# axiom-crypto/halo2-lib

Hardware: AMD Instinct MI355X
Metric: create_proof constraints/sec (k=19 ECDSA configuration, halo2-ecc/configs/secp256k1/bench_ecdsa.config:1); MSM G1-adds/sec in `msm_2_20` (higher is better)
Workload: dtype u32 (254-bit Montgomery integers as 8x32 / 9x29-bit limbs); 1 GPU; BASELINE configs[3]: h2hip_plonk_create_proof, k=19 secp256k1-ECDSA shape (bench_ecdsa.config:1: 1 advice + 1 lookup + 1 constants column, lookup_bits 18), synthetic circuit-like witness resident in HBM; 1 step = 1 proof, bytes back on the host; constraints_per_proof=524280, msm_count=12, msm_size=524288, extended_k=21, degree=5, proof_bytes=960

## Files before the change

### halo2-lib_amd/csrc/capi.hip

```cpp
#include <stdarg.h>

#include <algorithm>

#include "internal.h"
#include <sched.h>

namespace h2 {

static thread_local char g_err[512] = "";

void set_error(const char *fmt, ...) {
    va_list ap;
    va_start(ap, fmt);
    vsnprintf(g_err, sizeof(g_err), fmt, ap);
    va_end(ap);
}

int ws_reserve(h2hip_ctx *ctx, int slot, size_t bytes, void **out) {
    DevBuf &b = ctx->ws[slot];
    if (bytes == 0) bytes = 256;
    if (b.cap < bytes) {
        if (b.p) {
            H2_HIPCHK(hipStreamSynchronize(ctx->stream));
            if (ctx->clean_stream) H2_HIPCHK(hipStreamSynchronize(ctx->clean_stream));
// ... 135 lines not shown
    ctx->pending.clear();
}

static void prof_collect_all(h2hip_ctx *ctx);
void prof_fold_child(h2hip_ctx *parent, h2hip_ctx *child) {
    prof_collect(child);
    for (auto &kv : child->stats) {
        parent->stats[kv.first].total_ms += kv.second.total_ms;
        parent->stats[kv.first].launches += kv.second.launches;
        parent->stats[kv.first].spans.insert(parent->stats[kv.first].spans.end(), kv.second.spans.begin(), kv.second.spans.end());
    }
    child->stats.clear();
}
static void prof_collect_all(h2hip_ctx *ctx) {
    prof_collect(ctx);
    for (h2hip_ctx *l : ctx->lane)
        if (l) prof_fold_child(ctx, l);
}

}

using namespace h2;

extern "C" {

const char *h2hip_last_error(void) { return g_err; }
int h2hip_version(void) { return 100; }

int h2hip_device_count(int *count) {
    H2_REQUIRE(count, "count is NULL");
    int n = 0;
    hipError_t e = hipGetDeviceCount(&n);
    if (e != hipSuccess) {
        *count = 0;
        set_error("hipGetDeviceCount failed: %s", hipGetErrorString(e));
        return H2HIP_ERR_NO_DEVICE;
    }
    *count = n;
    return H2HIP_OK;
}

int h2hip_init(int device, void *hip_stream, h2hip_ctx **out) {
    H2_REQUIRE(out, "out is NULL");
    *out = nullptr;
    int n = 0;
    if (hipGetDeviceCount(&n) != hipSuccess || n <= 0) {
        set_error("no HIP device available (libh2hip has no CPU fallback)");
        return H2HIP_ERR_NO_DEVICE;
    }
    H2_REQUIRE(device >= 0 && device < n, "device index out of range");
    H2_HIPCHK(hipSetDevice(device));
    h2hip_ctx *ctx = new h2hip_ctx();
    ctx->device = device;
    hipDeviceProp_t prop;
    if (hipGetDeviceProperties(&prop, device) == hipSuccess) ctx->num_cus = prop.multiProcessorCount;
    if (hip_stream) {
        ctx->stream = (hipStream_t)hip_stream;
        ctx->own_stream = false;
    } else {
        hipError_t e = hipStreamCreateWithFlags(&ctx->stream, hipStreamNonBlocking);
        if (e != hipSuccess) {
            set_error("hipStreamCreate failed: %s", hipGetErrorString(e));
            delete ctx;
            return H2HIP_ERR_HIP;
        }
        ctx->own_stream = true;
    }
    *out = ctx;
    return H2HIP_OK;
}

}
namespace h2 {
constexpr size_t JOB_RING_BYTES = (size_t)1 << 20;
int upload_jobs(h2hip_ctx *ctx, void *dst_dev, const void *src_host, size_t bytes) {
    if (!bytes) return H2HIP_OK;
    if (bytes > JOB_RING_BYTES / 4) {
        H2_HIPCHK(hipMemcpyAsync(dst_dev, src_host, bytes, hipMemcpyHostToDevice, ctx->stream));
        H2_HIPCHK(hipStreamSynchronize(ctx->stream));
        return H2HIP_OK;
    }
    if (!ctx->job_ring) H2_HIPCHK(hipHostMalloc((void **)&ctx->job_ring, JOB_RING_BYTES, 0));
    const size_t need = (bytes + 255) / 256 * 256;
    if (ctx->job_ring_off + need > JOB_RING_BYTES) {
        H2_HIPCHK(hipStreamSynchronize(ctx->stream));
        ctx->job_ring_off = 0;
    }
    char *slot = ctx->job_ring + ctx->job_ring_off;
    memcpy(slot, src_host, bytes);
    ctx->job_ring_off += need;
    H2_HIPCHK(hipMemcpyAsync(dst_dev, slot, bytes, hipMemcpyHostToDevice, ctx->stream));
    return H2HIP_OK;
}
}
extern "C" {

void h2hip_destroy(h2hip_ctx *ctx) {
    if (!ctx) return;
    hipSetDevice(ctx->device);
    hipStreamSynchronize(ctx->stream);
    for (int l = 0; l < 4; ++l)
        if (ctx->lane[l]) hipStreamSynchronize(ctx->lane[l]->stream);
    if (ctx->clean_stream) {
        hipStreamSynchronize(ctx->clean_stream);
        hipStreamDestroy(ctx->clean_stream);
        hipEventDestroy(ctx->clean_ev);
        hipEventDestroy(ctx->clean_ev1);
        hipEventDestroy(ctx->used_ev);
    }
    if (ctx->tail_ev) hipEventDestroy(ctx->tail_ev);
    if (ctx->sorted_ev) hipEventDestroy(ctx->sorted_ev);
    if (ctx->job_ring) hipHostFree(ctx->job_ring);
    if (ctx->poll_host) hipHostFree(ctx->poll_host);
    for (auto &b : ctx->ws)
        if (b.p) hipFree(b.p);
    for (auto &t : ctx->twiddles) {
        hipFree(t.t1);
        hipFree(t.t2);
        for (int k = 0; k < 4; ++k) {
            if (t.direct[k]) hipFree(t.direct[k]);
        }
    }
    for (auto &p : ctx->pending) {
        hipEventDestroy(p.begin);
        hipEventDestroy(p.end);
    }
    for (auto e : ctx->event_pool) hipEventDestroy(e);
    if (ctx->prof_ref && ctx->own_prof_ref) hipEventDestroy(ctx->prof_ref);
    for (int l = 0; l < 4; ++l)
        if (ctx->lane[l]) {
            h2hip_destroy(ctx->lane[l]);
            hipEventDestroy(ctx->lane_ev[l]);
        }
    if (ctx->fork_ev) hipEventDestroy(ctx->fork_ev);
    if (ctx->fork_ev2) hipEventDestroy(ctx->fork_ev2);
    if (ctx->fork_ev3) hipEventDestroy(ctx->fork_ev3);
    for (auto e : ctx->timer_ev)
        if (e) hipEventDestroy(e);
    if (ctx->own_stream) hipStreamDestroy(ctx->stream);
    delete ctx;
}

int h2hip_sync(h2hip_ctx *ctx) {
    H2_DEVICE_GUARD(ctx);
    H2_REQUIRE(ctx, "ctx is NULL");
    H2_HIPCHK(hipStreamSynchronize(ctx->stream));
    return H2HIP_OK;
}

static int *param_slot(h2hip_ctx *ctx, const char *name) {
#define H2_KNOB_SLOT(knob, inherit, legal, domain) \
    if (!strcmp(name, #knob)) return &ctx->knob;
    H2_KNOB_TABLE(H2_KNOB_SLOT)
#undef H2_KNOB_SLOT
    return nullptr;
}
int h2hip_set_param(h2hip_ctx *ctx, const char *name, int value) {
    H2_DEVICE_GUARD(ctx);
    H2_REQUIRE(ctx && name, "NULL argument");
    int *p = param_slot(ctx, name);
    H2_REQUIRE(p, "unknown parameter name");
#define H2_KNOB_CHECK(knob, inherit, legal, domain)                                                     \
    if (p == &ctx->knob) {                                                                              \
        const int v = value;                                                                            \
        if (!(legal)) {                                                                                 \
            set_error("h2hip_set_param: invalid argument: " #knob " = %d: must be " domain, value);   \
            return H2HIP_ERR_INVALID;                                                                   \
        }                                                                                               \
    }
    H2_KNOB_TABLE(H2_KNOB_CHECK)
#undef H2_KNOB_CHECK
    *p = value;
    return H2HIP_OK;
}
int h2hip_get_param(h2hip_ctx *ctx, const char *name, int *value) {
    H2_DEVICE_GUARD(ctx);
    H2_REQUIRE(ctx && name && value, "NULL argument");
    int *p = param_slot(ctx, name);
    H2_REQUIRE(p, "unknown parameter name");
    *value = *p;
    return H2HIP_OK;
}

int h2hip_malloc(h2hip_ctx *ctx, size_t bytes, void **dptr) {
    H2_DEVICE_GUARD(ctx);
    H2_REQUIRE(ctx && dptr, "NULL argument");
    hipError_t e = hipMalloc(dptr, bytes ? bytes : 256);
    if (e != hipSuccess) {
        set_error("hipMalloc(%zu) failed: %s", bytes, hipGetErrorString(e));
        return H2HIP_ERR_NOMEM;
    }
    return H2HIP_OK;
}
int h2hip_free(h2hip_ctx *ctx, void *dptr) {
    H2_DEVICE_GUARD(ctx);
    H2_REQUIRE(ctx, "ctx is NULL");
    if (!dptr) return H2HIP_OK;
    H2_HIPCHK(hipStreamSynchronize(ctx->stream));
    H2_HIPCHK(hipFree(dptr));
    return H2HIP_OK;
}
int h2hip_host_register(h2hip_ctx *ctx, void *host_ptr, size_t bytes) {
    H2_DEVICE_GUARD(ctx);
    H2_REQUIRE(ctx && host_ptr && bytes, "NULL argument");
    H2_HIPCHK(hipHostRegister(host_ptr, bytes, hipHostRegisterDefault));
    return H2HIP_OK;
}
int h2hip_host_unregister(h2hip_ctx *ctx, void *host_ptr) {
    H2_DEVICE_GUARD(ctx);
    H2_REQUIRE(ctx && host_ptr, "NULL argument");
    H2_HIPCHK(hipHostUnregister(host_ptr));
    return H2HIP_OK;
}
int h2hip_upload(h2hip_ctx *ctx, void *dst_dev, const void *src_host, size_t bytes) {
    H2_DEVICE_GUARD(ctx);
    H2_REQUIRE(ctx && (bytes == 0 || (dst_dev && src_host)), "NULL argument");
    if (!bytes) return H2HIP_OK;
    H2_HIPCHK(hipMemcpyAsync(dst_dev, src_host, bytes, hipMemcpyHostToDevice, ctx->stream));
    H2_HIPCHK(hipStreamSynchronize(ctx->stream));
    return H2HIP_OK;
}
int h2hip_download(h2hip_ctx *ctx, void *dst_host, const void *src_dev, size_t bytes) {
    H2_DEVICE_GUARD(ctx);
    H2_REQUIRE(ctx && (bytes == 0 || (dst_host && src_dev)), "NULL argument");
    if (!bytes) return H2HIP_OK;
    H2_HIPCHK(hipMemcpyAsync(dst_host, src_dev, bytes, hipMemcpyDeviceToHost, ctx->stream));
    H2_HIPCHK(hipStreamSynchronize(ctx->stream));
    return H2HIP_OK;
}

int h2hip_profile_enable(h2hip_ctx *ctx, int on) {
    H2_DEVICE_GUARD(ctx);
    H2_REQUIRE(ctx, "ctx is NULL");
    prof_collect_all(ctx);
    ctx->profiling = on != 0;
    return H2HIP_OK;
}
int h2hip_profile_filter(h2hip_ctx *ctx, const char *prefix) {
    H2_DEVICE_GUARD(ctx);
    H2_REQUIRE(ctx, "ctx is NULL");
    prof_collect_all(ctx);
    ctx->prof_filter = prefix ? prefix : "";
    return H2HIP_OK;
}
int h2hip_profile_reset(h2hip_ctx *ctx) {
    H2_DEVICE_GUARD(ctx);
    H2_REQUIRE(ctx, "ctx is NULL");
    prof_collect_all(ctx);
    ctx->stats.clear();
    if (!ctx->prof_ref) {
        H2_HIPCHK(hipEventCreate(&ctx->prof_ref));
        ctx->own_prof_ref = true;
    }
    if (ctx->own_prof_ref) {
        H2_HIPCHK(hipEventRecord(ctx->prof_ref, ctx->stream));
        H2_HIPCHK(hipEventSynchronize(ctx->prof_ref));
    }
    return H2HIP_OK;
}
int h2hip_profile_get_busy(h2hip_ctx *ctx, const char *prefix, double *busy_ms) {
    H2_DEVICE_GUARD(ctx);
    H2_REQUIRE(ctx && prefix && busy_ms, "NULL argument");
    prof_collect_all(ctx);
    std::vector<std::pair<float, float>> all;
    size_t len = strlen(prefix);
    for (auto &kv : ctx->stats)
        if (kv.first.compare(0, len, prefix) == 0) all.insert(all.end(), kv.second.spans.begin(), kv.second.spans.end());
    std::sort(all.begin(), all.end());
    double busy = 0;
    float cur0 = 0, cur1 = -1;
    for (auto &sp : all) {
        if (cur1 < cur0 || sp.first > cur1) {
            if (cur1 >= cur0) busy += cur1 - cur0;
            cur0 = sp.first;
            cur1 = sp.second;
        } else if (sp.second > cur1) {
            cur1 = sp.second;
        }
    }
    if (cur1 >= cur0) busy += cur1 - cur0;
    *busy_ms = busy;
    return H2HIP_OK;
}
int h2hip_profile_get(h2hip_ctx *ctx, const char *prefix, double *total_ms, uint64_t *launches) {
    H2_DEVICE_GUARD(ctx);
    H2_REQUIRE(ctx && prefix, "NULL argument");
    prof_collect_all(ctx);
    double ms = 0;
    uint64_t cnt = 0;
    size_t len = strlen(prefix);
    for (auto &kv : ctx->stats)
        if (kv.first.compare(0, len, prefix) == 0) {
            ms += kv.second.total_ms;
            cnt += kv.second.launches;
        }
    if (total_ms) *total_ms = ms;
    if (launches) *launches = cnt;
    return H2HIP_OK;
}
int h2hip_profile_dump(h2hip_ctx *ctx, char *out, size_t cap, size_t *needed) {
    H2_DEVICE_GUARD(ctx);
    H2_REQUIRE(ctx && (out || cap == 0), "NULL argument");
    prof_collect_all(ctx);
    std::string text;
    for (auto &kv : ctx->stats) {
        std::vector<std::pair<float, float>> all(kv.second.spans.begin(), kv.second.spans.end());
        std::sort(all.begin(), all.end());
        double busy = 0;
        float cur0 = 0, cur1 = -1;
        for (auto &sp : all) {
            if (cur1 < cur0 || sp.first > cur1) {
                if (cur1 >= cur0) busy += cur1 - cur0;
                cur0 = sp.first;
                cur1 = sp.second;
            } else if (sp.second > cur1) {
                cur1 = sp.second;
            }
        }
        if (cur1 >= cur0) busy += cur1 - cur0;
        char line[256];
        snprintf(line, sizeof(line), "%s %.6f %llu %.6f\n", kv.first.c_str(), kv.second.total_ms, (unsigned long long)kv.second.launches, busy);
        text += line;
    }
// ... 31 lines not shown
```

### halo2-lib_amd/csrc/fr_ops.hip

```cpp
#include "internal.h"
#include "fr29.cuh"
#include "fq29.cuh"

namespace h2 {


enum { OP_ADD = 0, OP_SUB = 1, OP_MUL = 2 };

template <int OP>
__global__ __launch_bounds__(256) void fr_binop_kernel(Fr *__restrict__ out, const Fr *__restrict__ a, const Fr *__restrict__ b, size_t n) {
    size_t stride = (size_t)gridDim.x * blockDim.x;
    for (size_t i = (size_t)blockIdx.x * blockDim.x + threadIdx.x; i < n; i += stride) {
        Fr x = a[i], y = b[i];
        out[i] = OP == OP_ADD ? fe_add(x, y) : OP == OP_SUB ? fe_sub(x, y) : fe_mul(x, y);
    }
}

__global__ __launch_bounds__(256) void fr_mul_add_kernel(Fr *__restrict__ out, const Fr *__restrict__ a, const Fr *__restrict__ b,
                                                         const Fr *__restrict__ c, size_t n) {
    size_t stride = (size_t)gridDim.x * blockDim.x;
    for (size_t i = (size_t)blockIdx.x * blockDim.x + threadIdx.x; i < n; i += stride) out[i] = fe_add(fe_mul(a[i], b[i]), c[i]);
}

__global__ __launch_bounds__(256) void fr_axpby_kernel(Fr *__restrict__ y, Fr s, bool scale_y, const Fr *__restrict__ x, Fr a, size_t n) {
    size_t stride = (size_t)gridDim.x * blockDim.x;
    for (size_t i = (size_t)blockIdx.x * blockDim.x + threadIdx.x; i < n; i += stride) {
        Fr v = y[i];
        if (scale_y) v = fe_mul(v, s);
        if (x) v = fe_add(v, fe_mul(a, x[i]));
        y[i] = v;
    }
}

constexpr uint32_t LINCOMB_MAX = 15;
struct LinCombArgs {
    const Fr *p[LINCOMB_MAX];
    Fr29 c[LINCOMB_MAX];
    uint32_t count, accumulate;
};
__global__ __launch_bounds__(256) void fr_lincomb_kernel(Fr *out, LinCombArgs a, size_t n) {
    const size_t stride = (size_t)gridDim.x * blockDim.x;
    for (size_t i = (size_t)blockIdx.x * blockDim.x + threadIdx.x; i < n; i += stride) {
        Fr29 tot = a.accumulate ? f29_split<R29P>(out[i]) : Fr29::zero();
        for (uint32_t j0 = 0; j0 < a.count; j0 += 5) {
            Fr29 x[5], c[5];
#pragma unroll
            for (uint32_t t = 0; t < 5; ++t) {
                const bool live = j0 + t < a.count;
                x[t] = live ? f29_split<R29P>(a.p[j0 + t][i]) : Fr29::zero();
                c[t] = live ? a.c[j0 + t] : Fr29::zero();
            }
            tot = f29_add(tot, f29_dot<5>(x, c));
        }
        out[i] = f29_pack_canonical<FrP>(f29_weak_reduce(f29_norm(tot)));
    }
}

__global__ __launch_bounds__(256) void fr_batch_invert_kernel(const Fr *src, Fr *dst, Fr *__restrict__ scratch, size_t n) {
    const size_t T = (size_t)gridDim.x * blockDim.x, t = (size_t)blockIdx.x * blockDim.x + threadIdx.x;
    if (t >= n) return;
    Fr acc = Fr::one();
    size_t last = t;
    for (size_t i = t; i < n; i += T) {
        Fr v = src[i];
        scratch[i] = acc;
        if (!v.is_zero()) acc = fe_mul(acc, v);
        last = i;
    }
    Fr inv = fe_inv(acc);
    for (size_t i = last;; i -= T) {
        Fr v = src[i];
        if (!v.is_zero()) {
            dst[i] = fe_mul(inv, scratch[i]);
            inv = fe_mul(inv, v);
        } else if (dst != src) {
            dst[i] = v;
        }
        if (i < T) break;
    }
}


constexpr uint32_t SCAN_J = 8;
__global__ __launch_bounds__(256) void fr_prefix_prod_tile_kernel(const Fr *__restrict__ in, Fr *__restrict__ out, Fr *__restrict__ tile_prod,
                                                                  size_t n, size_t seg_stride) {
    __shared__ Fr sh[256];
    in += (size_t)blockIdx.y * seg_stride;
    out += (size_t)blockIdx.y * seg_stride;
    tile_prod += (size_t)blockIdx.y * gridDim.x;
    const uint32_t tid = threadIdx.x;
    const size_t base = ((size_t)blockIdx.x * 256 + tid) * SCAN_J;
    Fr acc = Fr::one();
    for (uint32_t k = 0; k < SCAN_J; ++k)
        if (base + k < n) acc = fe_mul(acc, in[base + k]);
    sh[tid] = acc;
    __syncthreads();
    for (uint32_t d = 1; d < 256; d <<= 1) {
        Fr o = Fr::one();
        if (tid >= d) o = sh[tid - d];
        __syncthreads();
        if (tid >= d) sh[tid] = fe_mul(sh[tid], o);
        __syncthreads();
    }
    Fr run = tid ? sh[tid - 1] : Fr::one();
    for (uint32_t k = 0; k < SCAN_J; ++k)
        if (base + k < n) {
            run = fe_mul(run, in[base + k]);
            out[base + k] = run;
        }
    if (tid == 255) tile_prod[blockIdx.x] = sh[255];
}
__global__ __launch_bounds__(1024) void fr_prefix_prod_sums_kernel(Fr *__restrict__ tile_prod, uint32_t ntiles) {
    __shared__ Fr sh[1024];
    tile_prod += (size_t)blockIdx.x * ntiles;
    const uint32_t tid = threadIdx.x;
    const uint32_t per = (ntiles + 1023) / 1024, lo = tid * per, hi = lo + per < ntiles ? lo + per : ntiles;
    Fr acc = Fr::one();
    for (uint32_t k = lo; k < hi; ++k) acc = fe_mul(acc, tile_prod[k]);
    sh[tid] = acc;
    __syncthreads();
    for (uint32_t d = 1; d < 1024; d <<= 1) {
        Fr o = Fr::one();
        if (tid >= d) o = sh[tid - d];
        __syncthreads();
        if (tid >= d) sh[tid] = fe_mul(sh[tid], o);
        __syncthreads();
    }
    Fr run = tid ? sh[tid - 1] : Fr::one();
    for (uint32_t k = lo; k < hi; ++k) {
        Fr t = tile_prod[k];
        tile_prod[k] = run;
        run = fe_mul(run, t);
    }
}
__global__ __launch_bounds__(256) void fr_prefix_prod_apply_kernel(Fr *__restrict__ out, const Fr *__restrict__ tile_excl, size_t n, size_t seg_stride) {
    const size_t base = ((size_t)blockIdx.x * 256 + threadIdx.x) * SCAN_J;
    if (blockIdx.x == 0) return;
    out += (size_t)blockIdx.y * seg_stride;
    Fr m = tile_excl[(size_t)blockIdx.y * gridDim.x + blockIdx.x];
    for (uint32_t k = 0; k < SCAN_J; ++k)
        if (base + k < n) out[base + k] = fe_mul(out[base + k], m);
}
__global__ __launch_bounds__(256) void fr_set_one_kernel(Fr *__restrict__ z) {
    if (threadIdx.x == 0 && blockIdx.x == 0) z[0] = Fr::one();
}
__global__ __launch_bounds__(256) void fr_ratio_rows_kernel(Fr *__restrict__ r, const Fr *__restrict__ num, const Fr *__restrict__ den_inv, size_t total,
                                                            size_t seg_len, int chained) {
    const size_t stride = (size_t)gridDim.x * blockDim.x;
    for (size_t g = (size_t)blockIdx.x * blockDim.x + threadIdx.x; g < total; g += stride) {
        const size_t seg = g / seg_len, i = g - seg * seg_len;
        const size_t dst = chained ? g + 1 : seg * (seg_len + 1) + i + 1;
        r[dst] = fe_mul(num[g], den_inv[g]);
        if (i == 0 && (!chained || seg == 0)) r[dst - 1] = Fr::one();
    }
}
struct RowPtrs {
    Fr *p[32];
};
__global__ __launch_bounds__(256) void fr_scatter_rows_kernel(RowPtrs dst, const Fr *__restrict__ src, size_t src_stride, size_t len) {
    Fr *__restrict__ d = dst.p[blockIdx.y];
    const Fr *__restrict__ sp = src + (size_t)blockIdx.y * src_stride;
    const size_t stride = (size_t)gridDim.x * blockDim.x;
    for (size_t i = (size_t)blockIdx.x * blockDim.x + threadIdx.x; i < len; i += stride) d[i] = sp[i];
}

}

using namespace h2;

extern "C" {

static int binop(h2hip_ctx *ctx, int op, void *out, const void *a, const void *b, size_t n) {
    H2_REQUIRE(ctx && (n == 0 || (out && a && b)), "NULL argument");
    if (!n) return H2HIP_OK;
    dim3 g(grid_for(ctx, n)), blk(256);
    prof_begin(ctx, "fr_binop_kernel");
    if (op == OP_ADD) hipLaunchKernelGGL(fr_binop_kernel<OP_ADD>, g, blk, 0, ctx->stream, (Fr *)out, (const Fr *)a, (const Fr *)b, n);
    if (op == OP_SUB) hipLaunchKernelGGL(fr_binop_kernel<OP_SUB>, g, blk, 0, ctx->stream, (Fr *)out, (const Fr *)a, (const Fr *)b, n);
    if (op == OP_MUL) hipLaunchKernelGGL(fr_binop_kernel<OP_MUL>, g, blk, 0, ctx->stream, (Fr *)out, (const Fr *)a, (const Fr *)b, n);
    prof_end(ctx);
    H2_HIPCHK(hipGetLastError());
    return H2HIP_OK;
}
int h2hip_fr_add_batch_dev(h2hip_ctx *ctx, void *out, const void *a, const void *b, size_t n) {
    H2_DEVICE_GUARD(ctx); return binop(ctx, OP_ADD, out, a, b, n); }
int h2hip_fr_sub_batch_dev(h2hip_ctx *ctx, void *out, const void *a, const void *b, size_t n) {
    H2_DEVICE_GUARD(ctx); return binop(ctx, OP_SUB, out, a, b, n); }
int h2hip_fr_mul_batch_dev(h2hip_ctx *ctx, void *out, const void *a, const void *b, size_t n) {
    H2_DEVICE_GUARD(ctx); return binop(ctx, OP_MUL, out, a, b, n); }
int h2hip_fr_mul_add_batch_dev(h2hip_ctx *ctx, void *out, const void *a, const void *b, const void *c, size_t n) {
    H2_DEVICE_GUARD(ctx);
    H2_REQUIRE(ctx && (n == 0 || (out && a && b && c)), "NULL argument");
    if (!n) return H2HIP_OK;
    prof_begin(ctx, "fr_mul_add_kernel");
    hipLaunchKernelGGL(fr_mul_add_kernel, dim3(grid_for(ctx, n)), dim3(256), 0, ctx->stream, (Fr *)out, (const Fr *)a, (const Fr *)b,
                       (const Fr *)c, n);
    prof_end(ctx);
    H2_HIPCHK(hipGetLastError());
    return H2HIP_OK;
}
int h2hip_fr_axpy_dev(h2hip_ctx *ctx, void *y, const void *a, const void *x, size_t n) {
    H2_DEVICE_GUARD(ctx);
    H2_REQUIRE(ctx && a && (n == 0 || (y && x)), "NULL argument");
    if (!n) return H2HIP_OK;
    Fr av;
    memcpy(&av, a, sizeof(Fr));
    prof_begin(ctx, "fr_axpby_kernel");
    hipLaunchKernelGGL(fr_axpby_kernel, dim3(grid_for(ctx, n)), dim3(256), 0, ctx->stream, (Fr *)y, Fr::one(), false, (const Fr *)x, av, n);
    prof_end(ctx);
    H2_HIPCHK(hipGetLastError());
    return H2HIP_OK;
}
int h2hip_fr_axpby_dev(h2hip_ctx *ctx, void *y, const void *s, const void *a, const void *x, size_t n) {
    H2_DEVICE_GUARD(ctx);
    H2_REQUIRE(ctx && a && s && (n == 0 || (y && x)), "NULL argument");
    if (!n) return H2HIP_OK;
    Fr av, sv;
    memcpy(&av, a, sizeof(Fr));
    memcpy(&sv, s, sizeof(Fr));
    prof_begin(ctx, "fr_axpby_kernel");
    hipLaunchKernelGGL(fr_axpby_kernel, dim3(grid_for(ctx, n)), dim3(256), 0, ctx->stream, (Fr *)y, sv, true, (const Fr *)x, av, n);
    prof_end(ctx);
    H2_HIPCHK(hipGetLastError());
    return H2HIP_OK;
}
int h2hip_fr_scale_dev(h2hip_ctx *ctx, void *y, const void *s, size_t n) {
    H2_DEVICE_GUARD(ctx);
    H2_REQUIRE(ctx && s && (n == 0 || y), "NULL argument");
    if (!n) return H2HIP_OK;
    Fr sv;
    memcpy(&sv, s, sizeof(Fr));
    prof_begin(ctx, "fr_axpby_kernel");
    hipLaunchKernelGGL(fr_axpby_kernel, dim3(grid_for(ctx, n)), dim3(256), 0, ctx->stream, (Fr *)y, sv, true, (const Fr *)nullptr, Fr::one(), n);
    prof_end(ctx);
    H2_HIPCHK(hipGetLastError());
    return H2HIP_OK;
}

int h2hip_fr_linear_combination_dev(h2hip_ctx *ctx, void *out, const void *const *polys, const void *coeffs, size_t count, size_t n) {
    H2_DEVICE_GUARD(ctx);
    H2_REQUIRE(ctx && (n == 0 || out) && (count == 0 || (polys && coeffs)), "NULL argument");
    if (!n) return H2HIP_OK;
    for (size_t j = 0; j < count; ++j) H2_REQUIRE(polys[j], "NULL polynomial");
    if (!count) {
        H2_HIPCHK(hipMemsetAsync(out, 0, sizeof(Fr) * n, ctx->stream));
        return H2HIP_OK;
    }
    const Fr *cs = (const Fr *)coeffs;
    for (size_t j0 = 0; j0 < count; j0 += LINCOMB_MAX) {
        LinCombArgs a;
        a.count = (uint32_t)(count - j0 < LINCOMB_MAX ? count - j0 : LINCOMB_MAX);
        a.accumulate = j0 ? 1u : 0u;
        for (uint32_t t = 0; t < LINCOMB_MAX; ++t) {
            const bool live = t < a.count;
            Fr c;
            if (live) memcpy(&c, cs + j0 + t, sizeof(Fr));
            a.p[t] = live ? (const Fr *)polys[j0 + t] : nullptr;
            a.c[t] = live ? fr29_from_sat(c) : Fr29::zero();
        }
        prof_begin(ctx, "fr_lincomb_kernel");
        hipLaunchKernelGGL(fr_lincomb_kernel, dim3(grid_for(ctx, n)), dim3(256), 0, ctx->stream, (Fr *)out, a, n);
        prof_end(ctx);
    }
    H2_HIPCHK(hipGetLastError());
    return H2HIP_OK;
}

}
namespace h2 {
int fr_batch_invert_to(h2hip_ctx *ctx, const Fr *src, Fr *dst, size_t n) {
    if (!n) return H2HIP_OK;
    Fr *scratch = nullptr;
    H2_CHK(ws_reserve(ctx, h2hip_ctx::WS_TMP1, sizeof(Fr) * n, (void **)&scratch));
    size_t per_lane = (size_t)ctx->fr_invert_run;
    if (per_lane < 1) {
        per_lane = n >> 16;
        per_lane = per_lane < 4 ? 4 : per_lane > 32 ? 32 : per_lane;
    }
    size_t lanes = (n + per_lane - 1) / per_lane;
    uint32_t blocks = (uint32_t)((lanes + 255) / 256);
    prof_begin(ctx, "fr_batch_invert_kernel");
    hipLaunchKernelGGL(fr_batch_invert_kernel, dim3(blocks), dim3(256), 0, ctx->stream, src, dst, scratch, n);
    prof_end(ctx);
    H2_HIPCHK(hipGetLastError());
    return H2HIP_OK;
}
}
extern "C" {
int h2hip_fr_batch_invert_dev(h2hip_ctx *ctx, void *a, size_t n) {
    H2_DEVICE_GUARD(ctx);
    H2_REQUIRE(ctx && (n == 0 || a), "NULL argument");
    return fr_batch_invert_to(ctx, (const Fr *)a, (Fr *)a, n);
}

static int prefix_product_segments(h2hip_ctx *ctx, const Fr *in, Fr *out, size_t n, size_t segments, size_t seg_stride) {
    const uint32_t tile = 256 * SCAN_J;
    uint32_t ntiles = (uint32_t)((n + tile - 1) / tile);
    H2_REQUIRE(segments >= 1 && segments <= 65535, "1..65535 segments");
    Fr *tp = nullptr;
    H2_CHK(ws_reserve(ctx, h2hip_ctx::WS_TMP2, sizeof(Fr) * ((size_t)ntiles * segments + 1), (void **)&tp));
    prof_begin(ctx, "fr_prefix_prod_kernels");
    hipLaunchKernelGGL(fr_prefix_prod_tile_kernel, dim3(ntiles, (uint32_t)segments), dim3(256), 0, ctx->stream, in, out, tp, n, seg_stride);
    hipLaunchKernelGGL(fr_prefix_prod_sums_kernel, dim3((uint32_t)segments), dim3(1024), 0, ctx->stream, tp, ntiles);
    hipLaunchKernelGGL(fr_prefix_prod_apply_kernel, dim3(ntiles, (uint32_t)segments), dim3(256), 0, ctx->stream, out, (const Fr *)tp, n, seg_stride);
    prof_end(ctx);
    H2_HIPCHK(hipGetLastError());
    return H2HIP_OK;
}
static int prefix_product_inplace(h2hip_ctx *ctx, const Fr *in, Fr *out, size_t n) { return prefix_product_segments(ctx, in, out, n, 1, 0); }
}
namespace h2 {
int fr_scatter_rows(h2hip_ctx *ctx, Fr *const *dst, size_t count, const Fr *src, size_t src_stride, size_t len) {
    if (!count || !len) return H2HIP_OK;
    prof_begin(ctx, "fr_scatter_rows_kernel");
    for (size_t s0 = 0; s0 < count; s0 += 32) {
        const uint32_t g = (uint32_t)(count - s0 < 32 ? count - s0 : 32);
        RowPtrs rows;
        for (uint32_t j = 0; j < 32; ++j) rows.p[j] = dst[s0 + (j < g ? j : 0)];
        hipLaunchKernelGGL(fr_scatter_rows_kernel, dim3(grid_for(ctx, len), g), dim3(256), 0, ctx->stream, rows, src + s0 * src_stride, src_stride, len);
    }
    prof_end(ctx);
    H2_HIPCHK(hipGetLastError());
    return H2HIP_OK;
}
}
extern "C" {
int h2hip_fr_prefix_product_dev(h2hip_ctx *ctx, void *out, const void *in, size_t n) {
    H2_DEVICE_GUARD(ctx);
    H2_REQUIRE(ctx && (n == 0 || (out && in)), "NULL argument");
    if (!n) return H2HIP_OK;
    return prefix_product_inplace(ctx, (const Fr *)in, (Fr *)out, n);
}
int h2hip_fr_grand_product_dev(h2hip_ctx *ctx, void *z, const void *num, const void *den, size_t n) {
    H2_DEVICE_GUARD(ctx);
    H2_REQUIRE(ctx && z && (n == 0 || (num && den)), "NULL argument");
    Fr *zz = (Fr *)z;
    hipLaunchKernelGGL(fr_set_one_kernel, dim3(1), dim3(64), 0, ctx->stream, zz);
    if (!n) return H2HIP_OK;
    Fr *t = nullptr;
    H2_CHK(ws_reserve(ctx, h2hip_ctx::WS_TMP0, sizeof(Fr) * n, (void **)&t));
    H2_CHK(fr_batch_invert_to(ctx, (const Fr *)den, t, n));
    H2_CHK(binop(ctx, OP_MUL, t, t, num, n));
    return prefix_product_inplace(ctx, t, zz + 1, n);
}

int h2hip_fr_grand_products_dev(h2hip_ctx *ctx, void *const *z, const void *num, const void *den, size_t segments, size_t seg_len, int chained) {
    H2_DEVICE_GUARD(ctx);
    H2_REQUIRE(ctx && (segments == 0 || z) && (segments == 0 || seg_len == 0 || (num && den)), "NULL argument");
    if (!segments) return H2HIP_OK;
    for (size_t s2 = 0; s2 < segments; ++s2) H2_REQUIRE(z[s2], "NULL product column");
    H2_REQUIRE(segments <= 65535 && seg_len < ((size_t)1 << 40), "too many segments");
    const size_t total = segments * seg_len;
    const size_t rlen = chained ? total + 1 : segments * (seg_len + 1);
    Fr *t = nullptr, *r = nullptr;
    H2_CHK(ws_reserve(ctx, h2hip_ctx::WS_TMP0, sizeof(Fr) * (total + 2 * rlen), (void **)&t));
    r = t + total;
    Fr *e = r + rlen;
    if (!total) {
        for (size_t s2 = 0; s2 < segments; ++s2) hipLaunchKernelGGL(fr_set_one_kernel, dim3(1), dim3(64), 0, ctx->stream, (Fr *)z[s2]);
        H2_HIPCHK(hipGetLastError());
        return H2HIP_OK;
    }
    H2_CHK(fr_batch_invert_to(ctx, (const Fr *)den, t, total));
    prof_begin(ctx, "fr_ratio_rows_kernel");
    hipLaunchKernelGGL(fr_ratio_rows_kernel, dim3(grid_for(ctx, total)), dim3(256), 0, ctx->stream, r, (const Fr *)num, (const Fr *)t, total, seg_len,
                       chained ? 1 : 0);
    prof_end(ctx);
    if (segments == 1) return prefix_product_segments(ctx, r, (Fr *)z[0], rlen, 1, 0);
    if (chained) H2_CHK(prefix_product_segments(ctx, r, e, rlen, 1, 0));
    else H2_CHK(prefix_product_segments(ctx, r, e, seg_len + 1, segments, seg_len + 1));
    return fr_scatter_rows(ctx, (Fr *const *)z, segments, e, chained ? seg_len : seg_len + 1, seg_len + 1);
}

}
```

### halo2-lib_amd/csrc/internal.h

```cpp
#pragma once
#include <hip/hip_runtime.h>
#include <stdint.h>
#include <stdio.h>
#include <string.h>
#include <functional>
#include <map>
#include <string>
#include <vector>

#include "../../include/h2hip.h"
#include "ec.cuh"
#include "ec29.cuh"

namespace h2 {

void set_error(const char *fmt, ...);

#define H2_HIPCHK(expr)                                                                              \
    do {                                                                                             \
        hipError_t e__ = (expr);                                                                     \
        if (e__ != hipSuccess) {                                                                     \
            h2::set_error("%s:%d: %s -> %s", __FILE__, __LINE__, #expr, hipGetErrorString(e__));     \
            return H2HIP_ERR_HIP;                                                                    \
        }                                                                                            \
    } while (0)

#define H2_CHK(expr)                      \
    do {                                  \
        int r__ = (expr);                 \
        if (r__ != H2HIP_OK) return r__;  \
    } while (0)

#define H2_REQUIRE_AS(func, cond, msg)                           \
    do {                                                         \
        if (!(cond)) {                                           \
            h2::set_error("%s: invalid argument: %s", func, msg); \
            return H2HIP_ERR_INVALID;                            \
        }                                                        \
    } while (0)
#define H2_REQUIRE(cond, msg) H2_REQUIRE_AS(__func__, cond, msg)

struct DevBuf {
    void *p = nullptr;
    size_t cap = 0;
};

struct TwiddleSet {
    uint32_t log_n = 0, lo_bits = 0;
    Fr omega;
    void *t1 = nullptr;
    void *t2 = nullptr;
    void *direct[4] = {nullptr, nullptr, nullptr, nullptr};
    uint32_t direct_log_s[4] = {0, 0, 0, 0};
};

struct KernelStat {
    double total_ms = 0;
    uint64_t launches = 0;
    std::vector<std::pair<float, float>> spans;
};

}

struct h2hip_ctx {
    int device = 0;
    hipStream_t stream = nullptr;
    bool own_stream = false;
    int num_cus = 256;
    enum { WS_NTT = 0, WS_DIGITS, WS_COUNTS, WS_OFFSETS, WS_CURSOR, WS_SKEY, WS_SVAL, WS_BUCKETS, WS_PKEY0, WS_PVAL0, WS_PKEY1,
           WS_PVAL1, WS_SEG, WS_WIN, WS_OUT, WS_SCAN, WS_TMP0, WS_TMP1, WS_TMP2, WS_STAGE, WS_POSEIDON, WS_FBTABLE, WS_BATCH, WS_LK0, WS_LK1, WS_LK2, WS_LK3, WS_LK4, WS_LK5, WS_VANISH, WS_BATCH_BUCKETS, WS_COUNT };
    h2::DevBuf ws[WS_COUNT];
    std::vector<h2::TwiddleSet> twiddles;
    uint32_t pos_t = 0, pos_rf = 0, pos_rp = 0;
    bool msm_lds_attr_set = false, lookup_lds_attr_set = false, ntt_lds_attr_set = false;
    int msm_window_bits = 0;
    int msm_chunk = 0;
    int msm_chunk_lone = -1;
    int msm_seg = 4;
    int msm_quad_tails = 1;
    int msm_quad_seg_max = 32768;
    int msm_sort_threads = 1024;
    int msm_sort_groups = 0;
    int msm_hist_split = 0;
    int msm_hist_packed = 1;
    int msm_scatter_split = 0;
    int msm_scatter_full_lds = 0;
    int msm_table_split = 1;
    int msm_lanes = 0;
    int msm_stagger_sorts = -1;
    int msm_fuse_cols = 0;
    int msm_defer_reduce = 1;
    int clean_on_lane = 1;
    int ntt_tile_bits = 10;
    int ntt_min_col_bits = 2;
    int ntt_full_table = 1;
    int ntt_tile_kernel = 1;
    int ntt_debug_skip = 0;
    int quotient_29 = 1;
    int kate_29 = 1;
    int kate_coeffs_per_lane = 0;
    int fr_invert_run = 0;
    int lookup_big_tile_bits = 19;
    int host_poll = 1;
#ifdef H2_HIPEMU
    int plonk_warm_keygen = 0;
#else
    int plonk_warm_keygen = 1;
#endif
    int plonk_tail_overlap = 1;
    int plonk_side_on_lanes = 1;
    int plonk_permute_in_commit = 1;
    int plonk_merge_products = 1;
    int plonk_shard_side = 1;
    int plonk_route_rows = 1;
    int plonk_lazy_upload = 1;
    int plonk_early_intt = 1;
    int plonk_gate_before_join = 0;
    bool is_lane = false;
    h2hip_ctx *lane[4] = {nullptr, nullptr, nullptr, nullptr};
    hipEvent_t lane_ev[4] = {nullptr, nullptr, nullptr, nullptr};
    hipEvent_t sorted_ev = nullptr;
    char *job_ring = nullptr;
    size_t job_ring_off = 0;
    hipEvent_t fork_ev = nullptr, fork_ev2 = nullptr, fork_ev3 = nullptr, tail_ev = nullptr;
    hipStream_t clean_stream = nullptr;
    hipEvent_t clean_ev = nullptr, clean_ev1 = nullptr, used_ev = nullptr;
    void *clean_ptr[2] = {nullptr, nullptr};
    size_t clean_bytes[2] = {0, 0};
    hipEvent_t timer_ev[2] = {nullptr, nullptr};
    char *poll_host = nullptr;
    char *poll_dev = nullptr;
    unsigned long long poll_seq = 0;
    bool profiling = false;
    std::string prof_filter;
    std::map<std::string, h2::KernelStat> stats;
    struct PendingLaunch {
        std::string name;
        hipEvent_t begin, end;
        bool ended;
    };
    std::vector<PendingLaunch> pending;
    std::vector<hipEvent_t> event_pool;
    hipEvent_t prof_ref = nullptr;
    bool own_prof_ref = false;
};

namespace h2 {
inline bool knob_pow2(int v) { return v > 0 && (v & (v - 1)) == 0; }
}
#define H2_INHERITED true
#define H2_PARENT_ONLY(why) false
#define H2_KNOB_TABLE(K)                                                                                                                          \
    K(msm_window_bits, H2_INHERITED, v == 0 || (v >= 4 && v <= 16), "0 (auto) or 4..16")                                                         \
    K(msm_chunk, H2_INHERITED, v == 0 || (v >= 2 && v <= 4096), "0 (auto) or 2..4096")                                                          \
    K(msm_chunk_lone, H2_INHERITED, v >= -1 && v <= 4096, "-1 (auto), 0 (the batch rule) or 1..4096")                                          \
    K(msm_seg, H2_INHERITED, h2::knob_pow2(v) && v <= 1024, "a power of two <= 1024")                                                          \
    K(msm_quad_tails, H2_INHERITED, v == 0 || v == 1, "0 or 1")                                                                                 \
    K(msm_quad_seg_max, H2_INHERITED, v >= 0, ">= 0")                                                                                           \
    K(msm_sort_threads, H2_INHERITED, v == 256 || v == 512 || v == 1024, "256, 512 or 1024")                                                   \
    K(msm_sort_groups, H2_INHERITED, v >= 0 && v <= 1024, "0 (auto) or 1..1024")                                                               \
    K(msm_hist_split, H2_INHERITED, v == 0 || (h2::knob_pow2(v) && v <= 64), "0 or a power of two <= 64")                                      \
    K(msm_hist_packed, H2_INHERITED, v == 0 || v == 1, "0 or 1")                                                                                \
    K(msm_scatter_split, H2_INHERITED, v == 0 || (h2::knob_pow2(v) && v <= 64), "0 (auto) or a power of two <= 64")                            \
    K(msm_scatter_full_lds, H2_INHERITED, v == 0 || v == 1, "0 or 1")                                                                           \
    K(msm_table_split, H2_INHERITED, v == 0 || v == 1, "0 or 1")                                                                                \
    K(msm_lanes, H2_PARENT_ONLY("read only by the batch driver, on the caller's context"), v >= 0 && v <= 4, "0 (auto) or 1..4")              \
    K(msm_stagger_sorts, H2_PARENT_ONLY("read only by the batch driver, on the caller's context"), v >= -1 && v <= 1, "-1 (auto), 0 or 1")     \
    K(msm_fuse_cols, H2_PARENT_ONLY("read only by the batch driver, on the caller's context"), v >= 0 && v <= (int)h2::MSM_MAX_COLS,           \
      "0 (auto) or 1..32")                                                                                                                        \
    K(msm_defer_reduce, H2_PARENT_ONLY("read only by the batch driver, on the caller's context"), v == 0 || v == 1, "0 or 1")                  \
    K(clean_on_lane, H2_PARENT_ONLY("read only by the batch driver, on the caller's context"), v == 0 || v == 1, "0 or 1")                     \
    K(ntt_tile_bits, H2_INHERITED, v >= 4 && v <= 10, "4..10")                                                                                  \
    K(ntt_min_col_bits, H2_INHERITED, v >= 0 && v <= 5, "0..5")                                                                                 \
    K(ntt_full_table, H2_INHERITED, v == 0 || v == 1, "0 or 1")                                                                                 \
    K(ntt_tile_kernel, H2_INHERITED, v == 0 || v == 1, "0 or 1")                                                                                \
    K(ntt_debug_skip, H2_INHERITED, v >= 0 && v <= 2, "0, 1 or 2")                                                                              \
    K(quotient_29, H2_INHERITED, v == 0 || v == 1, "0 or 1")                                                                                    \
    K(kate_29, H2_INHERITED, v == 0 || v == 1, "0 or 1")                                                                                        \
    K(kate_coeffs_per_lane, H2_INHERITED, v == 0 || v == 1 || v == 2 || v == 4 || v == 8, "0 (by length), 1, 2, 4 or 8")                       \
    K(fr_invert_run, H2_INHERITED, v >= 0 && v <= 1024, "0 (auto) or 1..1024")                                                                 \
    K(lookup_big_tile_bits, H2_INHERITED, v >= 12 && v <= 28, "12..28")                                                                         \
    K(host_poll, H2_INHERITED, v == 0 || v == 1, "0 or 1")                                                                                      \
    K(plonk_warm_keygen, H2_PARENT_ONLY("read only by h2hip_plonk_keygen"), v == 0 || v == 1, "0 or 1")                                       \
    K(plonk_tail_overlap, H2_PARENT_ONLY("read only by create_proof, on the caller's context"), v == 0 || v == 1, "0 or 1")                    \
    K(plonk_side_on_lanes, H2_PARENT_ONLY("read only by create_proof, on the caller's context"), v == 0 || v == 1, "0 or 1")                   \
    K(plonk_permute_in_commit, H2_PARENT_ONLY("read only by create_proof, on the caller's context"), v == 0 || v == 1, "0 or 1")               \
    K(plonk_merge_products, H2_PARENT_ONLY("read only by create_proof, on the caller's context"), v == 0 || v == 1, "0 or 1")                  \
    K(plonk_shard_side, H2_PARENT_ONLY("read only by create_proof, on the caller's context"), v >= 0 && v <= 2, "0, 1 or 2 (forced)")          \
    K(plonk_route_rows, H2_PARENT_ONLY("read only by create_proof, on the caller's context"), v == 0 || v == 1, "0 or 1")                      \
    K(plonk_lazy_upload, H2_PARENT_ONLY("read only by create_proof, on the caller's context"), v == 0 || v == 1, "0 or 1")                     \
    K(plonk_early_intt, H2_PARENT_ONLY("read only by create_proof, on the caller's context"), v == 0 || v == 1, "0 or 1")                      \
    K(plonk_gate_before_join, H2_PARENT_ONLY("read only by create_proof, on the caller's context"), v == 0 || v == 1, "0 or 1")

namespace h2 {
inline void inherit_knobs(h2hip_ctx *c, const h2hip_ctx *p) {
#define H2_KNOB_INHERIT(name, inherit, legal, domain) \
    if (inherit) c->name = p->name;
    H2_KNOB_TABLE(H2_KNOB_INHERIT)
#undef H2_KNOB_INHERIT
    c->profiling = p->profiling;
    c->prof_filter = p->prof_filter;
    c->prof_ref = p->prof_ref;
}
struct DeviceGuard {
    int prev = -1;
    bool switched = false;
    explicit DeviceGuard(const h2hip_ctx *c) {
        if (c && hipGetDevice(&prev) == hipSuccess && prev != c->device) switched = hipSetDevice(c->device) == hipSuccess;
    }
    ~DeviceGuard() {
        if (switched) hipSetDevice(prev);
    }
    DeviceGuard(const DeviceGuard &) = delete;
    DeviceGuard &operator=(const DeviceGuard &) = delete;
};
}
#define H2_DEVICE_GUARD(ctx) h2::DeviceGuard device_guard__(ctx)

struct h2hip_bases {
    h2::G1Affine *pts = nullptr;
    h2::G1Affine *pts29 = nullptr;
    bool split = false;
    size_t n = 0;
    uint32_t window_bits = 0;
    uint32_t tables = 1;
};

namespace h2 {
struct alignas(128) TableEntry29 {
    uint32_t x[9], y[9];
    uint32_t pad[14];
};
static_assert(sizeof(TableEntry29) == 128, "one entry per 128-byte line");
int ws_reserve(h2hip_ctx *ctx, int slot, size_t bytes, void **out);
inline uint32_t grid_for(const h2hip_ctx *ctx, size_t n, size_t per_lane = 1) {
    size_t blocks = (n / per_lane + 255) / 256, cap = (size_t)ctx->num_cus * 8;
    if (blocks > cap) blocks = cap;
    return (uint32_t)(blocks ? blocks : 1);
}
inline Fr ld_fr(const void *p) {
    Fr r;
    memcpy(&r, p, sizeof(Fr));
    return r;
}
struct OmegaTable;
int ntt_pow_table(h2hip_ctx *ctx, uint32_t log_n, const Fr &omega, OmegaTable *out);

void prof_begin(h2hip_ctx *ctx, const char *name);
void prof_end(h2hip_ctx *ctx);
bool prof_launch_events(h2hip_ctx *ctx, const char *name, hipEvent_t *start, hipEvent_t *stop);

int ntt_run(h2hip_ctx *ctx, Fr *a, uint32_t log_n, const Fr &omega, const Fr *in_override, uint64_t in_len, const Fr *in_scale3,
            const Fr *out_scale3);
int ntt_run_batch(h2hip_ctx *ctx, Fr *const *a, const Fr *const *in_override, size_t ncols, uint32_t log_n, const Fr &omega, uint64_t in_len,
                  const Fr *in_scale3, const Fr *out_scale3);
constexpr uint32_t LK_COMPRESS_MAX_EXPRS = 49, LK_COMPRESS_MAX_WIDTH = 5;
int lookup_compress_batch_dev(h2hip_ctx *ctx, const Fr *const *cols, Fr *const *out, uint32_t count, uint32_t width, size_t rows, const Fr &theta);
int fr_scatter_rows(h2hip_ctx *ctx, Fr *const *dst, size_t count, const Fr *src, size_t src_stride, size_t len);
int upload_jobs(h2hip_ctx *ctx, void *dst_dev, const void *src_host, size_t bytes);
int exclusive_scan_u32_segments(h2hip_ctx *ctx, const uint32_t *in, uint32_t *out, uint32_t n, uint32_t segments, size_t in_stride,
                                size_t out_stride);
int exclusive_scan_u32(h2hip_ctx *ctx, const uint32_t *in, uint32_t *out, uint32_t n);
int batch_normalize_jac(h2hip_ctx *ctx, const G1Jac *tmp, G1Affine *out, uint32_t n);
int msm_prepare_bases(h2hip_ctx *ctx, h2hip_bases *bases, bool precompute);
int msm_run(h2hip_ctx *ctx, const h2hip_bases *bases, const Fr *scalars_dev, size_t n, XYZZ *out_dev);
constexpr uint32_t MSM_MAX_COLS = 32;
int msm_run_cols(h2hip_ctx *ctx, const h2hip_bases *bases, const Fr *const *scalars_dev, uint32_t ncols, size_t n, XYZZ *out_dev,
                 XYZZ29 *ext_buckets, bool ext_buckets_zeroed = false, hipEvent_t sorted_ev = nullptr);
struct BatchMsmHooks {
    std::function<int(size_t)> col;
    std::function<int()> mid;
    size_t mid_after = 0;
    std::function<int(hipEvent_t ev)> tail;
};
int msm_batch(h2hip_ctx *ctx, const h2hip_bases *bases, const h2hip_bases *const *bases_per_col, const void *const *scalars_in, bool scalars_on_host,
              size_t n, size_t count, int point_format, void *out_host, const BatchMsmHooks *hooks);
bool buckets_prezeroed(h2hip_ctx *ctx, int which, const void *buf, size_t bytes);
int buckets_clean_after_use(h2hip_ctx *ctx, int which, void *buf, size_t bytes, hipStream_t on = nullptr);
int sync_stream(h2hip_ctx *ctx);
int sync_results(h2hip_ctx *ctx, void *dst_host, const void *src_dev, size_t bytes);
void prof_fold_child(h2hip_ctx *parent, h2hip_ctx *child);
int rng_chacha_fill_dev(h2hip_ctx *ctx, Fr *out_dev, size_t n, const uint8_t seed[32], int rounds, uint64_t first_block, hipStream_t stream);
int comm_reserve_allgather_dev(h2hip_comm *comm, size_t bytes);
int comm_reserve_alltoall_dev(h2hip_comm *c, size_t bytes);
int plonk_phased_layout(const h2hip_phased_circuit_params &pp, h2hip_plonk_shape *shape, std::vector<std::vector<int>> *phase_cols,
                        uint32_t challenges[H2HIP_MAX_PHASE], bool *phased, h2hip_base_circuit_params *bp, const h2hip_rlc_circuit_params *rlc = nullptr);
int msm_reduce_cols(h2hip_ctx *ctx, const h2hip_bases *bases, uint32_t window_bits, const XYZZ29 *buckets, uint32_t ncols, XYZZ *out_dev);
uint32_t lookup_padded_keys(uint32_t u);
int lookup_sort_keys_dev(h2hip_ctx *ctx, void *keys, uint32_t N);
struct WitnessCheckJob {
    uint32_t u = 0;
    std::vector<const Fr *> cols;
    std::vector<uint32_t> gate_adv, gate_q;
    std::vector<uint32_t> gate_report;
    uint32_t num_rlc_gates = 0;
    Fr rlc_gamma;
    std::vector<uint32_t> lk_in, lk_q;
    const void *table_sorted = nullptr;
    uint32_t dyn_width = 0;
    std::vector<uint32_t> dyn_in, dyn_tab;
    uint32_t num_lookups = 0;
    std::vector<uint32_t> perm_col;
    const uint16_t *sigma_c = nullptr;
    const uint32_t *sigma_r = nullptr;
};
constexpr uint32_t WC_NONE = 0xFFFFFFFFu;
int witness_check_run(h2hip_ctx *ctx, const WitnessCheckJob &job, h2hip_witness_failure *failures_out, size_t max_failures, size_t *num_failures);
}
```

Before: 38.66 million constraints/s.

## Fuse grand-product computation into tiled three-pass scan with per-tile inversion

Replaces the batch-invert, ratio and prefix-product pipeline for segmented grand products with three kernels. The first computes per-tile products of numerator and denominator, the second scans the tile totals and inverts only one denominator per thread, and the third rebuilds the row products in registers and shared memory and writes them straight into the product columns. This cuts full-length memory passes and the large workspace for the whole-column batch inversion, at the cost of more field multiplications per row and a new code path with zero-denominator handling. The new path is on by default through a new knob.

```diff
diff --git a/halo2-lib_amd/csrc/capi.hip b/halo2-lib_amd/csrc/capi.hip
--- a/halo2-lib_amd/csrc/capi.hip
+++ b/halo2-lib_amd/csrc/capi.hip
@@ -311,6 +311,7 @@
 #define H2_KNOB_SLOT(knob, inherit, legal, domain) \
     if (!strcmp(name, #knob)) return &ctx->knob;
     H2_KNOB_TABLE(H2_KNOB_SLOT)
+    H2_KNOB_TABLE_LATER(H2_KNOB_SLOT)
 #undef H2_KNOB_SLOT
     return nullptr;
 }
@@ -328,6 +329,7 @@
         }                                                                                               \
     }
     H2_KNOB_TABLE(H2_KNOB_CHECK)
+    H2_KNOB_TABLE_LATER(H2_KNOB_CHECK)
 #undef H2_KNOB_CHECK
     *p = value;
     return H2HIP_OK;
diff --git a/halo2-lib_amd/csrc/fr_ops.hip b/halo2-lib_amd/csrc/fr_ops.hip
--- a/halo2-lib_amd/csrc/fr_ops.hip
+++ b/halo2-lib_amd/csrc/fr_ops.hip
@@ -164,6 +164,150 @@
     for (size_t i = (size_t)blockIdx.x * blockDim.x + threadIdx.x; i < len; i += stride) d[i] = sp[i];
 }
 
+constexpr uint32_t GP_J = 4, GP_TILE = 256 * GP_J;
+template <uint32_t I, uint32_t N, class F>
+__device__ __forceinline__ void gp_for(F &&f) {
+    if constexpr (I < N) {
+        f(std::integral_constant<uint32_t, I>{});
+        gp_for<I + 1, N>(f);
+    }
+}
+__device__ __forceinline__ Fr gp_load(const Fr *__restrict__ p, size_t row, size_t seg_len) {
+    const Fr v = p[row < seg_len ? row : seg_len - 1];
+    return row < seg_len ? v : Fr::one();
+}
+__device__ __forceinline__ void gp_zero_rule(Fr &a, Fr &d) {
+    if (d.is_zero()) {
+        a = Fr::zero();
+        d = Fr::one();
+    }
+}
+constexpr uint32_t GP_STAGE_BYTES = GP_TILE * 32 + 256 * 16;
+__device__ __forceinline__ Fr *gp_slot(unsigned char *stage, uint32_t r) { return (Fr *)(stage + (size_t)r * 32 + (size_t)(r / GP_J) * 16); }
+__global__ __launch_bounds__(256) void fr_gp_tile_totals_kernel(const Fr *__restrict__ num, const Fr *__restrict__ den, Fr *__restrict__ tn,
+                                                                Fr *__restrict__ td, size_t seg_len) {
+    __shared__ Fr shn[256], shd[256];
+    const uint32_t tid = threadIdx.x;
+    const size_t seg_off = (size_t)blockIdx.y * seg_len, first = (size_t)blockIdx.x * GP_TILE + tid;
+    Fr pn = Fr::one(), pd = Fr::one();
+    for (uint32_t k = 0; k < GP_J; ++k) {
+        Fr a = gp_load(num + seg_off, first + k * 256, seg_len), d = gp_load(den + seg_off, first + k * 256, seg_len);
+        gp_zero_rule(a, d);
+        pn = fe_mul(pn, a);
+        pd = fe_mul(pd, d);
+    }
+    shn[tid] = pn;
+    shd[tid] = pd;
+    __syncthreads();
+    for (uint32_t w = 128; w; w >>= 1) {
+        if (tid < w) {
+            shn[tid] = fe_mul(shn[tid], shn[tid + w]);
+            shd[tid] = fe_mul(shd[tid], shd[tid + w]);
+        }
+        __syncthreads();
+    }
+    if (tid == 0) {
+        const size_t kt = (size_t)blockIdx.y * gridDim.x + blockIdx.x;
+        tn[kt] = shn[0];
+        td[kt] = shd[0];
+    }
+}
+__global__ __launch_bounds__(256) void fr_gp_tile_prefix_kernel(Fr *__restrict__ tn, Fr *__restrict__ td, size_t tiles) {
+    __shared__ Fr shn[256], shd[256];
+    tn += (size_t)blockIdx.x * tiles;
+    td += (size_t)blockIdx.x * tiles;
+    const uint32_t tid = threadIdx.x;
+    const size_t per = (tiles + 255) / 256, lo = (size_t)tid * per < tiles ? (size_t)tid * per : tiles, hi = lo + per < tiles ? lo + per : tiles;
+    Fr pn = Fr::one(), pd = Fr::one();
+    for (size_t k = lo; k < hi; ++k) {
+        pn = fe_mul(pn, tn[k]);
+        pd = fe_mul(pd, td[k]);
+    }
+    shn[tid] = pn;
+    shd[tid] = pd;
+    __syncthreads();
+    for (uint32_t w = 1; w < 256; w <<= 1) {
+        Fr on = Fr::one(), od = Fr::one();
+        if (tid >= w) {
+            on = shn[tid - w];
+            od = shd[tid - w];
+        }
+        __syncthreads();
+        if (tid >= w) {
+            shn[tid] = fe_mul(shn[tid], on);
+            shd[tid] = fe_mul(shd[tid], od);
+        }
+        __syncthreads();
+    }
+    if (lo >= hi) return;
+    Fr inv = fe_inv(shd[tid]);
+    for (size_t k = hi; k-- > lo;) {
+        const Fr t = td[k];
+        td[k] = inv;
+        inv = fe_mul(inv, t);
+    }
+    Fr run = tid ? shn[tid - 1] : Fr::one();
+    for (size_t k = lo; k < hi; ++k) {
+        const Fr t = tn[k];
+        tn[k] = run;
+        run = fe_mul(run, t);
+    }
+}
+__global__ __launch_bounds__(256) void fr_gp_rows_kernel(RowPtrs z, const Fr *__restrict__ num, const Fr *__restrict__ den,
+                                                                   const Fr *__restrict__ tn, const Fr *__restrict__ td_inv, size_t seg_len, size_t seg0,
+                                                                   int chained) {
+    __shared__ Fr shn[256], shd[256];
+    __shared__ __attribute__((aligned(16))) unsigned char stage[GP_STAGE_BYTES];
+    const uint32_t tid = threadIdx.x;
+    const size_t seg = seg0 + blockIdx.y, kt = seg * gridDim.x + blockIdx.x, first = (size_t)blockIdx.x * GP_TILE + tid;
+    Fr *__restrict__ zc = z.p[blockIdx.y];
+    Fr a[GP_J], d[GP_J];
+    gp_for<0, GP_J>([&](auto k) { *gp_slot(stage, k * 256 + tid) = gp_load(num + seg * seg_len, first + k * 256, seg_len); });
+    __syncthreads();
+    gp_for<0, GP_J>([&](auto k) { a[k] = *gp_slot(stage, tid * GP_J + k); });
+    __syncthreads();
+    gp_for<0, GP_J>([&](auto k) { *gp_slot(stage, k * 256 + tid) = gp_load(den + seg * seg_len, first + k * 256, seg_len); });
+    __syncthreads();
+    gp_for<0, GP_J>([&](auto k) {
+        d[k] = *gp_slot(stage, tid * GP_J + k);
+        gp_zero_rule(a[k], d[k]);
+    });
+    Fr next = d[GP_J - 1];
+    d[GP_J - 1] = Fr::one();
+    gp_for<1, GP_J>([&](auto k) {
+        a[k] = fe_mul(a[k - 1], a[k]);
+        const Fr t = d[GP_J - 1 - k];
+        d[GP_J - 1 - k] = fe_mul(d[GP_J - k], next);
+        next = t;
+    });
+    shn[tid] = a[GP_J - 1];
+    shd[255 - tid] = fe_mul(d[0], next);
+    __syncthreads();
+    for (uint32_t w = 1; w < 256; w <<= 1) {
+        Fr on = Fr::one(), od = Fr::one();
+        if (tid >= w) {
+            on = shn[tid - w];
+            od = shd[tid - w];
+        }
+        __syncthreads();
+        if (tid >= w) {
+            shn[tid] = fe_mul(shn[tid], on);
+            shd[tid] = fe_mul(shd[tid], od);
+        }
+        __syncthreads();
+    }
+    const Fr before = tn[kt];
+    Fr c = fe_mul(before, td_inv[kt]);
+    if (tid) c = fe_mul(c, shn[tid - 1]);
+    if (tid < 255) c = fe_mul(c, shd[254 - tid]);
+    gp_for<0, GP_J>([&](auto k) { *gp_slot(stage, tid * GP_J + k) = fe_mul(c, fe_mul(a[k], d[k])); });
+    __syncthreads();
+    gp_for<0, GP_J>([&](auto k) {
+        if (first + k * 256 < seg_len) zc[first + k * 256 + 1] = *gp_slot(stage, k * 256 + tid);
+    });
+    if (first == 0) zc[0] = chained && seg ? fe_mul(before, td_inv[kt - 1]) : Fr::one();
+}
+
 }
 
 using namespace h2;
@@ -344,6 +488,30 @@
     return prefix_product_inplace(ctx, t, zz + 1, n);
 }
 
+static int grand_products_fused(h2hip_ctx *ctx, Fr *const *z, const Fr *num, const Fr *den, size_t segments, size_t seg_len, int chained) {
+    const size_t ntiles = (seg_len + GP_TILE - 1) / GP_TILE, tiles = segments * ntiles;
+    Fr *tn = nullptr;
+    H2_CHK(ws_reserve(ctx, h2hip_ctx::WS_TMP2, sizeof(Fr) * 2 * tiles, (void **)&tn));
+    Fr *td = tn + tiles;
+    prof_begin(ctx, "fr_gp_tile_totals_kernel");
+    hipLaunchKernelGGL(fr_gp_tile_totals_kernel, dim3((uint32_t)ntiles, (uint32_t)segments), dim3(256), 0, ctx->stream, num, den, tn, td, seg_len);
+    prof_end(ctx);
+    prof_begin(ctx, "fr_gp_tile_prefix_kernel");
+    hipLaunchKernelGGL(fr_gp_tile_prefix_kernel, dim3(chained ? 1u : (uint32_t)segments), dim3(256), 0, ctx->stream, tn, td, chained ? tiles : ntiles);
+    prof_end(ctx);
+    prof_begin(ctx, "fr_gp_rows_kernel");
+    for (size_t s0 = 0; s0 < segments; s0 += 32) {
+        const uint32_t g = (uint32_t)(segments - s0 < 32 ? segments - s0 : 32);
+        RowPtrs rows;
+        for (uint32_t j = 0; j < 32; ++j) rows.p[j] = z[s0 + (j < g ? j : 0)];
+        hipLaunchKernelGGL(fr_gp_rows_kernel, dim3((uint32_t)ntiles, g), dim3(256), 0, ctx->stream, rows, num, den, (const Fr *)tn, (const Fr *)td, seg_len,
+                           s0, chained ? 1 : 0);
+    }
+    prof_end(ctx);
+    H2_HIPCHK(hipGetLastError());
+    return H2HIP_OK;
+}
+
 int h2hip_fr_grand_products_dev(h2hip_ctx *ctx, void *const *z, const void *num, const void *den, size_t segments, size_t seg_len, int chained) {
     H2_DEVICE_GUARD(ctx);
     H2_REQUIRE(ctx && (segments == 0 || z) && (segments == 0 || seg_len == 0 || (num && den)), "NULL argument");
@@ -351,16 +519,17 @@
     for (size_t s2 = 0; s2 < segments; ++s2) H2_REQUIRE(z[s2], "NULL product column");
     H2_REQUIRE(segments <= 65535 && seg_len < ((size_t)1 << 40), "too many segments");
     const size_t total = segments * seg_len;
+    if (!total) {
+        for (size_t s2 = 0; s2 < segments; ++s2) hipLaunchKernelGGL(fr_set_one_kernel, dim3(1), dim3(64), 0, ctx->stream, (Fr *)z[s2]);
+        H2_HIPCHK(hipGetLastError());
+        return H2HIP_OK;
+    }
+    if (ctx->fr_products_fused) return grand_products_fused(ctx, (Fr *const *)z, (const Fr *)num, (const Fr *)den, segments, seg_len, chained);
     const size_t rlen = chained ? total + 1 : segments * (seg_len + 1);
     Fr *t = nullptr, *r = nullptr;
     H2_CHK(ws_reserve(ctx, h2hip_ctx::WS_TMP0, sizeof(Fr) * (total + 2 * rlen), (void **)&t));
     r = t + total;
     Fr *e = r + rlen;
-    if (!total) {
-        for (size_t s2 = 0; s2 < segments; ++s2) hipLaunchKernelGGL(fr_set_one_kernel, dim3(1), dim3(64), 0, ctx->stream, (Fr *)z[s2]);
-        H2_HIPCHK(hipGetLastError());
-        return H2HIP_OK;
-    }
     H2_CHK(fr_batch_invert_to(ctx, (const Fr *)den, t, total));
     prof_begin(ctx, "fr_ratio_rows_kernel");
     hipLaunchKernelGGL(fr_ratio_rows_kernel, dim3(grid_for(ctx, total)), dim3(256), 0, ctx->stream, r, (const Fr *)num, (const Fr *)t, total, seg_len,
diff --git a/halo2-lib_amd/csrc/internal.h b/halo2-lib_amd/csrc/internal.h
--- a/halo2-lib_amd/csrc/internal.h
+++ b/halo2-lib_amd/csrc/internal.h
@@ -101,6 +101,7 @@
     int kate_coeffs_per_lane = 0;
     int fr_invert_run = 0;
     int lookup_big_tile_bits = 19;
+    int fr_products_fused = 1;
     int host_poll = 1;
 #ifdef H2_HIPEMU
     int plonk_warm_keygen = 0;
@@ -192,11 +193,14 @@
     K(plonk_early_intt, H2_PARENT_ONLY("read only by create_proof, on the caller's context"), v == 0 || v == 1, "0 or 1")                      \
     K(plonk_gate_before_join, H2_PARENT_ONLY("read only by create_proof, on the caller's context"), v == 0 || v == 1, "0 or 1")
 
+#define H2_KNOB_TABLE_LATER(K) K(fr_products_fused, H2_INHERITED, v == 0 || v == 1, "0 or 1")
+
 namespace h2 {
 inline void inherit_knobs(h2hip_ctx *c, const h2hip_ctx *p) {
 #define H2_KNOB_INHERIT(name, inherit, legal, domain) \
     if (inherit) c->name = p->name;
     H2_KNOB_TABLE(H2_KNOB_INHERIT)
+    H2_KNOB_TABLE_LATER(H2_KNOB_INHERIT)
 #undef H2_KNOB_INHERIT
     c->profiling = p->profiling;
     c->prof_filter = p->prof_filter;
```

After: 38.65 million constraints/s. About the same (-0.0%).
